# YamaguchiAtsushi/pointcloud_processor

Measured on AMD Instinct MI355X. Metric: ray-hit tests/sec + candidate poses/sec (whole node), 1M-pt terrain, higher is better.
Workload: dtype f64 march / f32 point test; 1 GPU; C2: 1M-pt L-shape excavation terrain, 1024x256 ray fan, 256 candidate poses per GPU; terrain_points=1001740, poses_total=256, num_candidates_lattice=348, parallelism=pose-shard x1

## Files before the change

### include/pcp_abi.h

```cpp
#ifndef PCP_ABI_H
#define PCP_ABI_H

#include <stddef.h>
#include <stdint.h>

#ifdef __cplusplus
extern "C" {
#endif

#define PCP_ABI_VERSION 2

enum pcp_status {
    PCP_OK = 0,
    PCP_E_INVALID = -1,
    PCP_E_HIP = -2,
    PCP_E_CAPACITY = -3,
    PCP_E_STATE = -4,
    PCP_E_NOMEM = -5
};

typedef struct pcp_ctx pcp_ctx;

typedef struct pcp_cloud_view {
    const void *data;
// ... 295 lines not shown
int pcp_step_table(double end, double *steps, uint64_t cap, uint64_t *n);

int pcp_debug_exclusive_scan(pcp_ctx *ctx, const uint32_t *in, uint64_t n, uint32_t *out);

typedef struct pcp_fine_geo {
    int32_t built;
    int32_t tile;
    int32_t skip;
    int32_t packed;
    int32_t nx, ny, nz;
    int32_t F, reach, fnx, fny, rz, tsteps;
    uint64_t n_points, n_records, n_entries;
    uint64_t start_off;
    uint64_t frec_bytes, wpts_bytes, pts_bytes;
    double ox, oy, oz, c, inv_c, r_q;
    double cf, inv_cf, R2;
    double zq;
    double clear_zt0, clear_c;
} pcp_fine_geo;
int pcp_debug_fine_copy(pcp_ctx *ctx, pcp_fine_geo *geo, void *frec, uint64_t frec_cap,
                        void *wpts, uint64_t wpts_cap, void *pts, uint64_t pts_cap);

typedef struct pcp_fine_pivot_geo {
    int32_t built;
    int32_t enabled;
    int32_t fnx, fny;
    int32_t tx, ty;
    uint64_t n_slots;
    uint64_t bytes;
    double ox, oy, cf;
} pcp_fine_pivot_geo;
int pcp_debug_fine_pivot(pcp_ctx *ctx, pcp_fine_pivot_geo *geo, void *piv, uint64_t piv_cap);

typedef struct pcp_index_info {
    uint64_t n_points;
    double cell;
    int32_t nx, ny, nz;
    int32_t fine_pivot;
    double bmin[3], bmax[3];
    int32_t scan_layout;
    int32_t fine_tile;
} pcp_index_info;
int pcp_terrain_info(pcp_ctx *ctx, pcp_index_info *info);

#ifdef __cplusplus
}
#endif
#endif
```

### pointcloud_processor_amd/_abi.py

```python
from __future__ import annotations

import ctypes as C
import os
from pathlib import Path

import numpy as np

_HERE = Path(__file__).resolve().parent
LIB_PATH = _HERE / "_lib" / "libpcp.so"

PCP_OK = 0
PCP_E_INVALID = -1
PCP_E_HIP = -2
PCP_E_CAPACITY = -3
PCP_E_STATE = -4
PCP_E_NOMEM = -5

MAX_STEPS = 4096

PCP_MEM_DEVICE_IN = 1
PCP_MEM_DEVICE_OUT = 2

F_RANGE_Z, F_FOV_Z, F_VIS_Z, F_RANGE_M, F_FOV_M, F_VIS_M = 1, 2, 4, 8, 16, 32

# ... 163 lines not shown
    ("pcp_raycast_fan_stamps", C.c_int, [_P, _P, C.c_uint64, C.POINTER(FanParams), _P]),
    ("pcp_raycast_fan_burst", C.c_int, [_P, _P, C.c_uint64, C.POINTER(FanParams), C.c_int,
                                        C.POINTER(C.c_double)]),
    ("pcp_raycast_fan_keys", C.c_int, [_P, _P, C.c_uint64, C.POINTER(FanParams), C.c_uint64,
                                       C.c_uint64, _P, _P, _P]),
    ("pcp_comm_unique_id", C.c_int, [_P]),
    ("pcp_comm_init_rank", C.c_int, [_P, C.c_int, _P, C.c_int]),
    ("pcp_comm_info", C.c_int, [_P, C.POINTER(C.c_int), C.POINTER(C.c_int)]),
    ("pcp_get_runtime_info", C.c_int, [C.POINTER(RuntimeInfo)]),
    ("pcp_raycast_fan_allreduce", C.c_int, [_P, _P, C.c_uint64, C.POINTER(FanParams), C.c_uint64,
                                            C.c_uint64, _P, _P, C.POINTER(C.c_int64),
                                            C.POINTER(C.c_double)]),
    ("pcp_score_poses_allreduce", C.c_int, [_P, _P, C.c_uint64, _P, C.POINTER(VlParams),
                                            C.c_uint64, C.c_uint64, _P, _P, _P,
                                            C.POINTER(VlReport), C.POINTER(C.c_double)]),
    ("pcp_score_poses_stats", C.c_int, [_P, _P, C.c_uint64, _P, C.POINTER(VlParams), _P]),
    ("pcp_score_matrix", C.c_int, [_P, _P, C.c_uint64, _P, C.POINTER(VlParams), _P, _P]),
    ("pcp_place_sensors", C.c_int, [_P, _P, C.c_uint64, _P, C.POINTER(VlParams),
                                    C.POINTER(PlaceParams), _P, _P, _P, _P, _P, _P, _P, _P, _P]),
    ("pcp_place_pair", C.c_int, [_P, _P, C.c_uint64, _P, C.POINTER(VlParams),
                                 C.POINTER(PairParams), _P, _P, _P, _P, _P, _P, _P, _P, _P, _P,
                                 _P, _P, _P]),
    ("pcp_place_pair_burst", C.c_int, [_P, _P, C.c_uint64, _P, C.POINTER(VlParams),
                                       C.POINTER(PairParams), C.c_int, C.POINTER(C.c_double)]),
    ("pcp_simulate_scan", C.c_int, [_P, _P, C.c_uint64, C.POINTER(FanParams), _P, C.c_uint64,
                                    C.POINTER(C.c_uint64), _P, _P, _P, _P, _P, C.c_uint64,
                                    C.POINTER(C.c_uint64), _P, C.POINTER(C.c_uint64)]),
    ("pcp_simulate_scan_burst", C.c_int, [_P, _P, C.c_uint64, C.POINTER(FanParams), C.c_int,
                                          _P]),
    ("pcp_debug_exclusive_scan", C.c_int, [_P, _P, C.c_uint64, _P]),
    ("pcp_debug_fine_copy", C.c_int, [_P, C.POINTER(FineGeo), _P, C.c_uint64, _P, C.c_uint64, _P,
                                      C.c_uint64]),
    ("pcp_debug_fine_pivot", C.c_int, [_P, C.POINTER(FinePivotGeo), _P, C.c_uint64]),
    ("pcp_score_poses_burst", C.c_int, [_P, _P, C.c_uint64, _P, C.POINTER(VlParams), C.c_int,
                                        C.POINTER(C.c_double)]),
    ("pcp_stream_create", C.c_int, [_P, C.POINTER(_P)]),
    ("pcp_stream_destroy", C.c_int, [_P, _P]),
    ("pcp_step_table", C.c_int, [C.c_double, _P, C.c_uint64, C.POINTER(C.c_uint64)]),
    ("pcp_terrain_info", C.c_int, [_P, C.POINTER(IndexInfo)]),
    ("pcp_multi_create", C.c_int, [C.c_int, _P, C.POINTER(_P)]),
    ("pcp_multi_destroy", None, [_P]),
    ("pcp_multi_last_error", C.c_char_p, [_P]),
    ("pcp_multi_info", C.c_int, [_P, C.POINTER(C.c_int), C.POINTER(C.c_int)]),
    ("pcp_multi_ctx", _P, [_P, C.c_int]),
    ("pcp_multi_set_terrain", C.c_int, [_P, C.POINTER(CloudView)]),
    ("pcp_multi_set_aux_cloud", C.c_int, [_P, C.POINTER(CloudView)]),
    ("pcp_multi_set_cells", C.c_int, [_P, _P, _P, C.c_uint64]),
    ("pcp_multi_raycast_fan", C.c_int, [_P, _P, C.c_uint64, C.POINTER(FanParams), _P, _P,
                                        C.POINTER(C.c_int64)]),
    ("pcp_multi_score_poses", C.c_int, [_P, _P, C.c_uint64, _P, C.POINTER(VlParams), _P, _P,
                                        _P, C.POINTER(VlReport)]),
]
ABI_SYMBOLS = [s[0] for s in _SIGS]

_lib = None


def load_library(path: str | os.PathLike | None = None) -> C.CDLL:
    global _lib
    if _lib is not None and path is None:
        return _lib
    p = Path(path) if path else Path(os.environ.get("PCP_LIB", LIB_PATH))
    if not p.exists():
        raise OSError(f"libpcp.so not found at {p}: run __graft_entry__.build() "
                      f"(make -C pointcloud_processor_amd/csrc)")
    lib = C.CDLL(str(p), mode=C.RTLD_GLOBAL)
# ... 562 lines not shown
    def debug_exclusive_scan(self, a: np.ndarray) -> np.ndarray:
        a = np.ascontiguousarray(a, np.uint32)
        out = np.zeros(a.size + 1, np.uint32)
        self._check(self.lib.pcp_debug_exclusive_scan(self.h, _ptr(a), a.size, _ptr(out)),
                    "pcp_debug_exclusive_scan")
        return out

    def debug_fine_copy(self):
        geo = FineGeo()
        self._check(self.lib.pcp_debug_fine_copy(self.h, C.byref(geo), None, 0, None, 0, None, 0),
                    "pcp_debug_fine_copy")
        d = {k: getattr(geo, k) for k, _ in geo._fields_}
        if not geo.built:
            return d, None, None, None
        frec = np.zeros(geo.frec_bytes, np.uint8)
        wpts = np.zeros(geo.wpts_bytes, np.uint8)
        pts = np.zeros((geo.n_points, 4), np.float32)
        self._check(self.lib.pcp_debug_fine_copy(self.h, C.byref(geo), _ptr(frec), frec.nbytes,
                                                 _ptr(wpts), wpts.nbytes, _ptr(pts), pts.nbytes),
                    "pcp_debug_fine_copy")
        return d, frec, wpts, pts

    def debug_fine_pivot(self):
        geo = FinePivotGeo()
        self._check(self.lib.pcp_debug_fine_pivot(self.h, C.byref(geo), None, 0),
                    "pcp_debug_fine_pivot")
        d = {k: getattr(geo, k) for k, _ in geo._fields_}
        if not geo.built:
            return d, None
        piv = np.zeros((geo.n_slots, 3), np.float32)
        self._check(self.lib.pcp_debug_fine_pivot(self.h, C.byref(geo), _ptr(piv), piv.nbytes),
                    "pcp_debug_fine_pivot")
        return d, piv

    def score_matrix(self, poses5, zx120_pose5, params: VlParams):
        poses = np.ascontiguousarray(poses5, np.float64).reshape(-1, 5)
        zx = np.ascontiguousarray(zx120_pose5, np.float64)
        C_ = self.cells_count()
        P = poses.shape[0]
        sm = np.zeros((max(P, 1), max(C_, 1)), np.float64)
        sz = np.zeros(max(C_, 1), np.float64)
        self._check(self.lib.pcp_score_matrix(self.h, _ptr(poses), P, _ptr(zx), C.byref(params),
                                              _ptr(sm), _ptr(sz)), "pcp_score_matrix")
        return sm[:P, :C_].copy(), sz[:C_].copy()

    def place_sensors(self, poses5, zx120_pose5, params: VlParams, k_max: int,
                      min_separation: float = 0.0, want_round_totals: bool = False,
                      want_cells: bool = False, reserved: int = 0) -> dict:
        poses = np.ascontiguousarray(poses5, np.float64).reshape(-1, 5)
        zx = np.ascontiguousarray(zx120_pose5, np.float64)
        P = poses.shape[0]
        pp = PlaceParams(int(k_max), int(reserved), float(min_separation))
        kk = max(min(int(k_max), PLACE_MAX), 1)
        sel = np.full(kk, -1, np.int64)
        tot = np.zeros(kk, np.float64)
        cov = np.zeros(kk, np.int32)
        rt = np.zeros((kk, max(P, 1)), np.float64) if want_round_totals else None
        C_ = self.cells_count() if want_cells else 0
        cs = np.zeros(max(C_, 1), np.float64) if want_cells else None
        co = np.zeros(max(C_, 1), np.int32) if want_cells else None
        zt, zc, ns = C.c_double(), C.c_int32(), C.c_int32()
        self._check(self.lib.pcp_place_sensors(self.h, _ptr(poses) if P else None, P, _ptr(zx),
                                               C.byref(params), C.byref(pp), _ptr(sel), _ptr(tot),
                                               _ptr(cov), _ptr(rt), _ptr(cs), _ptr(co),
                                               C.byref(zt), C.byref(zc), C.byref(ns)),
                    "pcp_place_sensors")
# ... 310 lines not shown
```

### pointcloud_processor_amd/_stamps.py

```python
from __future__ import annotations

import hashlib
import os
from pathlib import Path

ROOT = Path(__file__).resolve().parents[1]
CSRC = ROOT / "pointcloud_processor_amd" / "csrc"
_COMMON = ["pcp_internal.hpp", "Makefile", "../../include/pcp_abi.h"]
WORKLOAD_SOURCES = {
    "fan": ["pcp_vlidar.hip", "pcp_fine.hip", "pcp_index.hip", "pcp_stencil.hpp",
            "pcp_grid.hpp", "pcp_fan_clear.hpp", "pcp_fan_clip.hpp", "pcp_fan_pivot.hpp"] + _COMMON,
    "filter": ["pcp_filter.hip", "pcp_rigid.hpp"] + _COMMON,
    "cells": ["pcp_vlidar.hip", "pcp_fine.hip", "pcp_index.hip", "pcp_stencil.hpp",
              "pcp_grid.hpp", "pcp_fan_clear.hpp", "pcp_fan_clip.hpp", "pcp_fan_pivot.hpp"] + _COMMON,
}


def workload_stamp(key: str) -> str:
    h = hashlib.sha256(os.environ.get("EXTRA", "").encode())
    for name in WORKLOAD_SOURCES[key]:
        f = (CSRC / name).resolve()
        h.update(name.encode())
        h.update(f.read_bytes())
    return h.hexdigest()[:16]
```

### pointcloud_processor_amd/csrc/pcp_context.hip

```cpp
#include <cmath>
#include <cstdio>
#include <dlfcn.h>
#include <execinfo.h>
#include <cstdarg>
#include <cstdlib>
#include <cstring>
#include <new>

#include "pcp_fan_clip.hpp"
#include "pcp_internal.hpp"

namespace pcp {

int set_err(pcp_ctx *ctx, int code, const char *fmt, ...) {
    if (ctx) {
        char buf[512];
        va_list ap;
        va_start(ap, fmt);
        vsnprintf(buf, sizeof(buf), fmt, ap);
        va_end(ap);
        ctx->err = buf;
    }
    return code;
}
// ... 564 lines not shown
int pcp_alloc_stats(uint64_t *device_reallocs, uint64_t *pinned_reallocs, uint64_t *bytes) {
    if (device_reallocs) *device_reallocs = alloc_count(0);
    if (pinned_reallocs) *pinned_reallocs = alloc_count(1);
    if (bytes) *bytes = alloc_count(2);
    return PCP_OK;
}

int pcp_device_count(int *n) {
    if (!n) return PCP_E_INVALID;
    int c = 0;
    if (hipGetDeviceCount(&c) != hipSuccess) c = 0;
    *n = c;
    return PCP_OK;
}

int pcp_create(int device, pcp_ctx **out) {
    if (!out) return PCP_E_INVALID;
    *out = nullptr;
    int c = 0;
    if (hipGetDeviceCount(&c) != hipSuccess || c <= 0) return PCP_E_HIP;
    if (device < 0 || device >= c) return PCP_E_INVALID;
    if (hipSetDevice(device) != hipSuccess) return PCP_E_HIP;
    pcp_ctx *ctx = new (std::nothrow) pcp_ctx();
    if (!ctx) return PCP_E_NOMEM;
    ctx->device = device;
    if (const char *fb = std::getenv("PCP_FAN_BATCH")) ctx->fan_batch = std::atoi(fb);
    if (const char *fw = std::getenv("PCP_FAN_NPW")) {
        const int v = std::atoi(fw);
        ctx->fan_npw = (v == 2 || v == 4 || v == 8 || v == 16 || v == 32) ? v : 1;
    }
    if (const char *fc = std::getenv("PCP_FAN_CULL")) ctx->fan_cull = std::atoi(fc) != 0;
    if (const char *cl = std::getenv("PCP_FAN_CLEAR")) ctx->terrain.fan_clear = std::atoi(cl) != 0;
    if (const char *pv = std::getenv("PCP_FAN_PIVOT")) ctx->terrain.fan_pivot = std::atoi(pv) != 0;
    if (const char *cp = std::getenv("PCP_FAN_CLIP"))
        ctx->terrain.fan_clip_e = std::atoi(cp) != 0 ? pcp::kClipSlack : pcp::kClipSlackWhole;
    if (const char *fo = std::getenv("PCP_FAN_ORDER")) ctx->fan_horizon_first = std::atoi(fo) != 0;
    if (const char *ho = std::getenv("PCP_FAN_HOST_OUT")) ctx->fan_host_out = std::atoi(ho) != 0;
    if (const char *ne = std::getenv("PCP_NORMALS_EXACT")) ctx->normals_exact = std::atoi(ne) != 0;
    if (const char *sw = std::getenv("PCP_SCORE_WIDE")) ctx->score_wide = std::atoi(sw) != 0;
    if (const char *wr = std::getenv("PCP_SCORE_WIDE_RAYS")) ctx->score_wide_rays = std::atoll(wr);
    if (const char *wg = std::getenv("PCP_SCORE_WIDE_G")) {
        char *end = nullptr;
        const long v = std::strtol(wg, &end, 10);
        if (end == wg || *end != '\0' || !(v == 2 || v == 4 || v == 8 || v == 16)) {
            std::fprintf(stderr, "libpcp: pcp_create: PCP_SCORE_WIDE_G=\"%s\" is not one of 2, 4, 8, 16\n",
                         wg);
            delete ctx;
            return PCP_E_INVALID;
        }
        ctx->score_wide_g = (int)v;
    }
    if (const char *co = std::getenv("PCP_CELLS_ORDER_FREE")) ctx->cells_all_ordered = std::atoi(co) == 0;
    if (const char *nbk = std::getenv("PCP_NB_BLOCKS")) ctx->nb_blocks = std::atoi(nbk);
    if (const char *sp = std::getenv("PCP_SCAN_ONEPASS")) ctx->scan_onepass = std::atoi(sp) != 0;
    if (const char *ip = std::getenv("PCP_INDEX_PAIR")) ctx->index_pair = std::atoi(ip) != 0;
    if (const char *as = std::getenv("PCP_AREA_STREAM")) ctx->area_side = std::atoi(as) != 0;
    if (const char *ns = std::getenv("PCP_NB_SMALL")) ctx->nb_small = std::atoi(ns) != 0;
    if (const char *rp = std::getenv("PCP_NB_REGION_PCT"))
        ctx->nb_region_pct = std::min(100, std::max(1, std::atoi(rp)));
    if (const char *gw = std::getenv("PCP_NB_GUESS_WORDS"))
        ctx->nb_guess_max = std::max<uint64_t>(1, std::strtoull(gw, nullptr, 10));
    if (const char *ct = std::getenv("PCP_COPY_THREADS")) ctx->copy_threads = std::atoi(ct);
    if (const char *fo = std::getenv("PCP_FM_HOST_OUT")) ctx->fm_host_out = std::atoi(fo) != 0;
    if (const char *ff = std::getenv("PCP_FM_FAST")) {
        const int v = std::atoi(ff);
        ctx->fm_fast = (v == 0 || v == 1) ? v : 2;
// ... 214 lines not shown
```

### pointcloud_processor_amd/csrc/pcp_fine.hip

```cpp
#pragma clang fp contract(off)

#include <cfloat>
#include <cmath>

#include <rocprim/device/device_radix_sort.hpp>

#include "pcp_fan_clear.hpp"
#include "pcp_fan_pivot.hpp"
#include "pcp_grid.hpp"
#include "pcp_internal.hpp"

namespace pcp {

namespace {

constexpr int kThreads = 256;

struct FineGeo {
    double ox, oy;
    double cf, inv_cf;
    double R2;
    int32_t fnx, fny;
    int32_t reach;
};

__device__ __forceinline__ bool in_window(const FineGeo &f, double px, double py, int wx, int wy) {
    const double x0 = f.ox + (double)wx * f.cf, y0 = f.oy + (double)wy * f.cf;
    const double dx = fmax(fmax(x0 - px, px - (x0 + f.cf)), 0.0);
    const double dy = fmax(fmax(y0 - py, py - (y0 + f.cf)), 0.0);
    return dx * dx + dy * dy <= f.R2;
}

__device__ __forceinline__ void fine_cell(const FineGeo &f, float x, float y, int &cx, int &cy) {
    cx = min(max((int)floor(((double)x - f.ox) * f.inv_cf), 0), f.fnx - 1);
    cy = min(max((int)floor(((double)y - f.oy) * f.inv_cf), 0), f.fny - 1);
}

__global__ void __launch_bounds__(kThreads)
k_zkeys(const float4 *__restrict__ pts, uint32_t n, unsigned long long *__restrict__ key,
// ... 165 lines not shown
    const uint32_t w = blockIdx.x * kThreads + threadIdx.x;
    if (w >= nw) return;
    const int x = (int)(w % (uint32_t)fnx), y = (int)(w / (uint32_t)fnx);
    uint32_t top = rz;
    for (int d = 0; d <= kClearMax && top > 0u; ++d) {
        const int ya = y - d, yb = y + d;
        const uint32_t la = ya >= 0 ? lev[(size_t)ya * fnx + x] : 0xFFFFFFFFu;
        const uint32_t lb = yb < fny ? lev[(size_t)yb * fnx + x] : 0xFFFFFFFFu;
        const uint32_t m = min(la, lb);
        for (uint32_t iz = m; iz < top; ++iz) h[(size_t)iz * nw + w] = (uint16_t)d;
        top = min(top, m);
    }
    for (uint32_t iz = 0; iz < top; ++iz) h[(size_t)iz * nw + w] = (uint16_t)(kClearMax + 1);
}

__global__ void __launch_bounds__(kThreads)
k_clear_code(const uint16_t *__restrict__ h, int fnx, int fny, uint32_t nw, uint32_t tx,
             size_t plane, uint16_t *__restrict__ fband) {
    const uint32_t w = blockIdx.x * kThreads + threadIdx.x, iz = blockIdx.y;
    if (w >= nw) return;
    const uint32_t wx = w % (uint32_t)fnx, wy = w / (uint32_t)fnx;
    if (fan_clear_border(wx, wy, iz, (uint32_t)fnx, (uint32_t)fny, gridDim.y)) return;
    const size_t r = (size_t)iz * plane + (((size_t)((wy >> 3) * tx + (wx >> 3)) << 6) |
                                           ((wy & 7u) << 3) | (wx & 7u));
    if (fband[r] != 0x00FFu) return;
    const uint16_t *row = h + (size_t)iz * nw + (size_t)wy * fnx;
    int D = (int)row[wx];
    for (int d = 1; d < D; ++d) {
        const int xa = (int)wx - d, xb = (int)wx + d;
        if (xa >= 0) D = min(D, max((int)row[xa], d));
        if (xb < fnx) D = min(D, max((int)row[xb], d));
    }
    fband[r] = (uint16_t)(0x00FFu | (fan_clear_code((uint32_t)D) << 8));
}

__global__ void __launch_bounds__(kThreads)
k_pivot(const float4 *__restrict__ wpts, const uint32_t *__restrict__ cstart, FineGeo f,
        uint32_t tx, uint32_t nslot, float *__restrict__ piv) {
    const uint32_t t = blockIdx.x * kThreads + threadIdx.x;
    if (t >= nslot) return;
    const uint32_t tile = t >> 6, sub = t & 63u;
    const uint32_t wx = (tile % tx) * 8u + (sub & 7u), wy = (tile / tx) * 8u + (sub >> 3);
    float3 best = make_float3(__int_as_float(0x7FC00000), __int_as_float(0x7FC00000), -INFINITY);
    if (wx < (uint32_t)f.fnx && wy < (uint32_t)f.fny) {
        const uint32_t w = wx + (uint32_t)f.fnx * wy;
        const uint32_t s = cstart[w] + w, e = cstart[w + 1] + w;
        PivotKey kb{};
        for (uint32_t j = s; j < e; ++j) {
            const float4 p = wpts[j];
            const PivotKey k{pivot_d2(f.ox, f.oy, f.cf, wx, wy, p.x, p.y), p.z,
                             __float_as_uint(p.w)};
            if (j == s || pivot_better(k, kb)) {
                kb = k;
                best = make_float3(p.x, p.y, p.z);
            }
        }
    }
    float *o = piv + 3 * (size_t)t;
    o[0] = best.x;
    o[1] = best.y;
    o[2] = best.z;
}

__global__ void __launch_bounds__(kThreads)
k_pack3(const float4 *__restrict__ src, uint32_t n, float *__restrict__ dst) {
    const uint32_t i = blockIdx.x * kThreads + threadIdx.x;
// ... 138 lines not shown
    hipLaunchKernelGGL(k_frec, dim3((unsigned)((nthr + kThreads - 1) / kThreads)), dim3(kThreads), 0,
                       st, went, (const uint32_t *)cstart, m, g.c, (uint32_t)fnx,
                       (uint32_t)fny, (uint32_t)rz, tsteps, tile, skip2 ? 1 : 0,
                       g.frec.as<uint2>(),
                       g.frec.as<uint16_t>(),
                       reinterpret_cast<uint32_t *>(g.frec.as<char>() + band_bytes));
    PCP_CHECK_LAUNCH(ctx);
    if (pivots) {
        hipLaunchKernelGGL(k_pivot, dim3((unsigned)((plan.npiv + kThreads - 1) / kThreads)),
                           dim3(kThreads), 0, st, (const float4 *)went, (const uint32_t *)cstart,
                           f, pivot_tiles((uint32_t)fnx), (uint32_t)plan.npiv,
                           g.fpiv.as<float>());
        PCP_CHECK_LAUNCH(ctx);
    }
    if (tile == 2) {
        const size_t lev_bytes = ((size_t)nw * 4 + 255) & ~(size_t)255;
        PCP_HIP(ctx, ctx->scratch[5].ensure(lev_bytes + (size_t)nw * rz * 2 + 64));
        uint32_t *lev = ctx->scratch[5].as<uint32_t>();
        uint16_t *hcol = reinterpret_cast<uint16_t *>(ctx->scratch[5].as<char>() + lev_bytes);
        const ClearGeo cg = plan.cg;
        PCP_HIP(ctx, hipMemsetAsync(lev, 0xFF, (size_t)nw * 4, st));
        hipLaunchKernelGGL(k_clear_level, dim3(gridn), dim3(kThreads), 0, st, pts, n, f, cg,
                           (int)rz, lev);
        PCP_CHECK_LAUNCH(ctx);
        const dim3 cgrid((unsigned)((nw + kThreads - 1) / kThreads), (unsigned)rz);
        hipLaunchKernelGGL(k_clear_col, dim3(cgrid.x), dim3(kThreads), 0, st,
                           (const uint32_t *)lev, (int)fnx, (int)fny, (uint32_t)nw, (uint32_t)rz,
                           hcol);
        PCP_CHECK_LAUNCH(ctx);
        hipLaunchKernelGGL(k_clear_code, cgrid, dim3(kThreads), 0, st, (const uint16_t *)hcol,
                           (int)fnx, (int)fny, (uint32_t)nw, (uint32_t)((fnx + 7) / 8), (size_t)(nrec / rz),
                           g.frec.as<uint16_t>());
        PCP_CHECK_LAUNCH(ctx);
    }
    if (pack) {
        hipLaunchKernelGGL(k_pack3, dim3((unsigned)((nent + kThreads - 1) / kThreads)),
                           dim3(kThreads), 0, st, (const float4 *)went, (uint32_t)nent,
                           g.wpts.as<float>());
        PCP_CHECK_LAUNCH(ctx);
    }
    g.wpack = pack ? 1 : 0;
    g.frx = (uint32_t)fnx;
    g.fry = (uint32_t)fny;
    g.frz = (uint32_t)rz;
    g.ffine = (float)F;
    g.ftile = tile;
    g.fskip = skip2 ? 2 : 1;
    g.fstart_off = tile == 2 ? band_bytes : 0;
    g.fnent = nent;
    g.fpiv_ok = pivots;
    g.fine_ok = true;
    return PCP_OK;
}

}

extern "C" int pcp_debug_fine_copy(pcp_ctx *ctx, pcp_fine_geo *geo, void *frec,
                                   uint64_t frec_cap, void *wpts, uint64_t wpts_cap, void *pts,
                                   uint64_t pts_cap) {
    using namespace pcp;
    if (!ctx || !geo) return PCP_E_INVALID;
    const GridIndex &g = ctx->terrain;
    *geo = pcp_fine_geo{};
    if (!g.present || !g.fine_ok) return PCP_OK;
    const FinePlan p = fine_plan(g, (int)g.ffine, g.ftile);
    geo->built = 1;
// ... 37 lines not shown
    if (frec) PCP_HIP(ctx, hipMemcpy(frec, g.frec.p, geo->frec_bytes, hipMemcpyDeviceToHost));
    if (wpts) PCP_HIP(ctx, hipMemcpy(wpts, g.wpts.p, geo->wpts_bytes, hipMemcpyDeviceToHost));
    if (pts) PCP_HIP(ctx, hipMemcpy(pts, g.pts.p, geo->pts_bytes, hipMemcpyDeviceToHost));
    return PCP_OK;
}

extern "C" int pcp_debug_fine_pivot(pcp_ctx *ctx, pcp_fine_pivot_geo *geo, void *piv,
                                    uint64_t piv_cap) {
    using namespace pcp;
    if (!ctx || !geo) return PCP_E_INVALID;
    const GridIndex &g = ctx->terrain;
    *geo = pcp_fine_pivot_geo{};
    if (!g.present || !g.fine_ok || !g.fpiv_ok) return PCP_OK;
    const FinePlan p = fine_plan(g, (int)g.ffine, g.ftile);
    geo->built = 1;
    geo->enabled = g.fan_pivot ? 1 : 0;
    geo->fnx = p.f.fnx;
    geo->fny = p.f.fny;
    geo->tx = (int32_t)pivot_tiles((uint32_t)p.fnx);
    geo->ty = (int32_t)pivot_tiles((uint32_t)p.fny);
    geo->n_slots = p.npiv;
    geo->bytes = p.npiv * kPivotBytes;
    geo->ox = p.f.ox;
    geo->oy = p.f.oy;
    geo->cf = p.f.cf;
    if (!piv) return PCP_OK;
    if (piv_cap < geo->bytes)
        return set_err(ctx, PCP_E_CAPACITY, "pcp_debug_fine_pivot: the buffer is too small");
    PCP_HIP(ctx, hipSetDevice(ctx->device));
    PCP_HIP(ctx, hipStreamSynchronize(ctx->stream));
    PCP_HIP(ctx, hipMemcpy(piv, g.fpiv.p, geo->bytes, hipMemcpyDeviceToHost));
    return PCP_OK;
}
```

### pointcloud_processor_amd/csrc/pcp_index.hip

```cpp
#include <cfloat>
#include <cmath>
#include <cstring>

#include "pcp_internal.hpp"
#include "pcp_grid.hpp"

namespace pcp {

constexpr uint64_t kMaxCells = 1ull << 25;
constexpr int kThreads = 256;

GridView GridIndex::view() const {
    GridView v{};
    v.pts = pts.as<const float4>();
    v.start = start.as<const uint32_t>();
    v.occ2 = occ2_ok ? occ2.as<const uint32_t>() : nullptr;
    v.c = c;
    v.inv_c = c > 0 ? 1.0 / c : 0.0;
    v.ox = bmin[0] - c;
    v.oy = bmin[1] - c;
    v.oz = bmin[2] - c;
    const double rm = r_q + kQueryMargin;
    double amax = 0.0;
    for (int a = 0; a < 3; ++a) amax = fmax(amax, fmax(fabs(bmin[a]), fabs(bmax[a])));
// ... 2 lines not shown
    v.lo_y = v.oy + rm;
    v.lo_z = v.oz + rm;
    v.nx = nx;
    v.ny = ny;
    v.nz = nz;
    v.n_pts = (uint32_t)n_pts;
    v.bx0 = bmin[0] - rb;
    v.bx1 = bmax[0] + rb;
    v.by0 = bmin[1] - rb;
    v.by1 = bmax[1] + rb;
    v.bz0 = bmin[2] - rb;
    v.bz1 = bmax[2] + rb;
    v.flo_x = (float)v.lo_x;
    v.flo_y = (float)v.lo_y;
    v.flo_z = (float)v.lo_z;
    v.finv_c = (float)v.inv_c;
    v.fnx1 = (float)(nx - 1);
    v.fny1 = (float)(ny - 1);
    v.fnz1 = (float)(nz - 1);
    const double bb[6] = {v.bx0, v.bx1, v.by0, v.by1, v.bz0, v.bz1};
    for (int a = 0; a < 6; ++a) v.fb[a] = (float)bb[a];
    v.occz = occz_ok ? occz.as<const uint16_t>() : nullptr;
    v.bstart = blk_ok ? bstart.as<const uint32_t>() : nullptr;
    v.bpts = blk_ok ? bpts.as<const float4>() : nullptr;
    v.fzoff = (float)(rm * v.inv_c);
    v.fzt = (float)((r_q + 2e-3) * v.inv_c);
    v.frec = fine_ok ? frec.as<const uint2>() : nullptr;
    v.wpts = fine_ok ? wpts.as<const float4>() : nullptr;
    v.frx = fine_ok ? frx : 0u;
    v.fry = fine_ok ? fry : 0u;
    v.frz = fine_ok ? frz : 0u;
    v.ffine = fine_ok ? ffine : 0.0f;
    v.ftile = fine_ok ? ftile : 0;
    v.fband = (fine_ok && ftile == 2) ? frec.as<const uint16_t>() : nullptr;
    v.fzc = (float)c;
    v.wpack = fine_ok ? wpack : 0;
    v.fzo = (float)v.oz;
    v.fstart = (fine_ok && ftile == 2)
                   ? reinterpret_cast<const uint32_t *>(frec.as<const char>() + fstart_off)
                   : nullptr;
    v.fus_off = (float)(rm * v.inv_c / (double)kZq);
    v.fskip = fine_ok ? fskip : 1;
    v.fclear = (fine_ok && ftile == 2 && fan_clear) ? 1 : 0;
    v.fclr_cf = fine_ok ? (float)(c / (double)ffine) : 0.0f;
    v.fclr_rb = std::nextafter((float)rb, INFINITY);
    const bool piv = fine_ok && ftile == 2 && fpiv_ok;
    v.fpiv = (piv && fan_pivot) ? fpiv.as<const float>() : nullptr;
    v.fptx = piv ? (frx + 7u) >> 3 : 0u;
    v.fpty = piv ? (fry + 7u) >> 3 : 0u;
    v.fclip_e = fan_clip_e;
    return v;
}

float exit_dist(float r2) {
    float d = std::sqrt(r2);
    while (d * d < r2) d = std::nextafter(d, INFINITY);
    for (float p = std::nextafter(d, 0.0f); p * p >= r2; p = std::nextafter(d, 0.0f)) d = p;
    return d;
}

__device__ __forceinline__ float ld_f32(const unsigned char *base, uint32_t off) {
    return *reinterpret_cast<const float *>(base + off);
}

__global__ void __launch_bounds__(kThreads)
k_extract(const unsigned char *__restrict__ raw, uint64_t n, uint32_t step, uint32_t ox,
          uint32_t oy, uint32_t oz, float4 *__restrict__ xyz, float *__restrict__ part,
// ... 510 lines not shown
    PCP_HIP(ctx, ctx->scratch[4].ensure(scan_tmp_bytes(ncm) + (ncm + 1) * sizeof(uint32_t)));
    if (int rc = exclusive_scan_u32_pair(ctx, cnt_a, ga.start.as<uint32_t>(), nca, cnt_a, cnt_b,
                                         gb.start.as<uint32_t>(), ncb, cnt_b, ctx->scratch[4].p,
                                         true))
        return rc;
    ctx->cell_cnt_dirty = ctx->cell_cnt2_dirty = false;
    PCP_HIP(ctx, ga.pts.ensure((size_t)nfin * sizeof(float4)));
    PCP_HIP(ctx, gb.pts.ensure((size_t)nfin * sizeof(float4)));
    hipLaunchKernelGGL(k_cell_place2, dim3(gridn), dim3(kThreads), 0, st,
                       ctx->scratch[0].as<const float4>(), n, (const uint2 *)cr_a,
                       ga.start.as<const uint32_t>(), ga.pts.as<float4>(), (const uint2 *)cr_b,
                       gb.start.as<const uint32_t>(), gb.pts.as<float4>());
    PCP_CHECK_LAUNCH(ctx);
    ga.present = gb.present = true;
    *paired = true;
    return PCP_OK;
}

int build_index(pcp_ctx *ctx, GridIndex &g, const pcp_cloud_view &v, double r_q, bool zsort,
                bool occ, const unsigned char **raw_io, unsigned char *raw_copy) {
    const uint64_t n = v.n;
    hipStream_t st = ctx->stream;
    if (n >= (1ull << 28))
        return set_err(ctx, PCP_E_INVALID, "index cloud of %llu points exceeds 2^28",
                       (unsigned long long)n);
    ProfScope prof(ctx, PCP_K_INDEX_BUILD);
    g.present = false;
    g.occz_ok = false;
    g.occ2_ok = false;
    g.blk_ok = false;
    g.blk_fail = false;
    g.fine_ok = false;
    g.fpiv_ok = false;
    g.fine_fail = false;
    const uint64_t raw_bytes = n * (uint64_t)v.point_step;
    const unsigned char *raw = raw_io ? *raw_io : nullptr;
    bool pinned = false;
    if (!raw && n && ctx->zc_in && raw_bytes <= kPinDirectMax) {
        const HostPiece pc{0, v.data, raw_bytes};
        const void *dv = nullptr;
        if (int rc0 = pin_stage(ctx, &pc, 1, raw_bytes, &dv)) return rc0;
        raw = static_cast<const unsigned char *>(dv);
        pinned = true;
    }
    if (!raw) {
        PCP_HIP(ctx, ctx->stage.ensure(raw_bytes));
        if (int rc0 = upload_async(ctx, ctx->stage.p, v.data, raw_bytes, st)) return rc0;
        raw = ctx->stage.as<unsigned char>();
    }
    const bool host_bb = n <= kHostBboxMax;
    const bool fuse_copy = raw_copy && host_bb && n && (v.point_step & 15u) == 0 &&
                           v.point_step <= 64 &&
                           ((reinterpret_cast<uintptr_t>(raw) | reinterpret_cast<uintptr_t>(raw_copy)) & 15u) == 0;
    if (raw_copy && n && !fuse_copy) {
        if (int rc0 = copy_pinned_async(ctx, raw_copy, raw, raw_bytes, st)) return rc0;
        raw = raw_copy;
    }
    if (raw_io) *raw_io = raw_copy && n ? raw_copy : raw;
    auto release_raw = [&]() {
        if (pinned && !raw_io) pin_release(ctx, st);
    };
    const int nb = (int)std::min<uint64_t>((n + kThreads - 1) / kThreads, 1024);
    PCP_HIP(ctx, ctx->scratch[0].ensure(n * sizeof(float4)));
    PCP_HIP(ctx, ctx->scratch[1].ensure((size_t)nb * 6 * sizeof(float) + 64 + nb * 4));
    PCP_HIP(ctx, ctx->stats_d.ensure(64));
    float *part = ctx->scratch[1].as<float>();
// ... 225 lines not shown
```

### pointcloud_processor_amd/csrc/pcp_internal.hpp

```cpp
#pragma once

#include <hip/hip_runtime.h>

#include <algorithm>
#include <atomic>
#include <cstdint>
#include <cstdio>
#include <string>
#include <vector>

#include "pcp_abi.h"
#include "pcp_fan_pick.hpp"

namespace pcp {
struct CopyPool;

constexpr double kPi = 3.14159265358979323846;
constexpr double kMinDistance = 0.5;
constexpr double kRayStep = 0.3;
constexpr double kVisRadius = 0.08;
constexpr double kRayRadius = kVisRadius * 0.7;
constexpr double kRelaxedRadius = kVisRadius * 3.0;
constexpr double kMinElevation = -85.0 * kPi / 180.0;
constexpr double kMaxElevation = 85.0 * kPi / 180.0;
// ... 65 lines not shown
    double bx0, bx1, by0, by1, bz0, bz1;
    float flo_x, flo_y, flo_z, finv_c;
    float fnx1, fny1, fnz1;
    float fb[6];
    const uint16_t *occz;
    float fzoff, fzt;
    const uint32_t *bstart;
    const float4 *bpts;
    const uint2 *frec;
    const float4 *wpts;
    uint32_t frx, fry, frz;
    float fus_off, ffine;
    int32_t ftile;
    const uint16_t *fband;
    const uint32_t *fstart;
    int32_t fskip;
    float fzc, fzo;
    int32_t wpack;
    int32_t fclear;
    float fclr_cf, fclr_rb;
    const float *fpiv;
    uint32_t fptx, fpty;
    float fclip_e;
};
constexpr float kZq = 2.0f / 250.0f;

struct GridIndex {
    bool present = false;
    uint64_t n_pts = 0;
    double r_q = 0.0;
    double c = 0.0;
    int32_t nx = 0, ny = 0, nz = 0;
    double bmin[3] = {0, 0, 0}, bmax[3] = {0, 0, 0};
    DevBuf pts, start, occ2, occz, bstart, bpts, frec, wpts, fpiv;
    bool occz_ok = false;
    bool blk_ok = false;
    bool blk_fail = false;
    bool fine_ok = false;
    bool fine_fail = false;
    uint32_t frx = 0, fry = 0, frz = 0;
    int32_t wpack = 0;
    float ffine = 0.0f;
    int32_t ftile = 0;
    int32_t fskip = 1;
    bool fan_clear = true;
    bool fpiv_ok = false;
    bool fan_pivot = true;
    float fan_clip_e = 1.0f / 64.0f;
    size_t fstart_off = 0;
    uint64_t fnent = 0;
    bool occ2_ok = false;
    GridView view() const;
    void release() {
        pts.release();
        start.release();
        occ2.release();
        occz.release();
        bstart.release();
        bpts.release();
        frec.release();
        wpts.release();
        fpiv.release();
        fpiv_ok = false;
        occz_ok = false;
        blk_ok = false;
        blk_fail = false;
        fine_ok = false;
        fine_fail = false;
        occ2_ok = false;
        present = false;
        n_pts = 0;
    }
};

struct ProfSlot {
    double total_ms = 0.0;
    uint64_t launches = 0;
};

struct CloudBufs {
    DevBuf xyz, idx, keys[2], sparse, sparse_idx, hist, out;
    DevBuf skeys;
    void release() {
        skeys.release();
        xyz.release();
        idx.release();
        for (int q = 0; q < 2; ++q) keys[q].release();
        sparse.release();
        sparse_idx.release();
        hist.release();
        out.release();
    }
};

struct PendingEvent {
    int kid;
// ... 289 lines not shown
```

Before: 7180 billion ray-hit tests/s.

## Build per-column tight z-band table so fan rays skip empty z slices

Adds a build-time kernel that, for each fine column and z layer, computes the actual z extent that points can reach within the query radius. It stores the narrowed band in a second buffer, which the ray-march view uses in place of the coarse band when enabled (on by default). Tighter bands should let the ray test skip more z sub-steps per cell. The cost is extra index-build work and memory, and the result is only correct if the band margin (rho + mu) is conservative enough.

```diff
diff --git a/include/pcp_abi.h b/include/pcp_abi.h
--- a/include/pcp_abi.h
+++ b/include/pcp_abi.h
@@ -351,6 +351,9 @@
 } pcp_fine_pivot_geo;
 int pcp_debug_fine_pivot(pcp_ctx *ctx, pcp_fine_pivot_geo *geo, void *piv, uint64_t piv_cap);
 
+int pcp_debug_fine_band(pcp_ctx *ctx, uint64_t *bytes, int32_t *enabled, void *band,
+                        uint64_t band_cap);
+
 typedef struct pcp_index_info {
     uint64_t n_points;
     double cell;
diff --git a/pointcloud_processor_amd/_abi.py b/pointcloud_processor_amd/_abi.py
--- a/pointcloud_processor_amd/_abi.py
+++ b/pointcloud_processor_amd/_abi.py
@@ -219,6 +219,8 @@
     ("pcp_debug_fine_copy", C.c_int, [_P, C.POINTER(FineGeo), _P, C.c_uint64, _P, C.c_uint64, _P,
                                       C.c_uint64]),
     ("pcp_debug_fine_pivot", C.c_int, [_P, C.POINTER(FinePivotGeo), _P, C.c_uint64]),
+    ("pcp_debug_fine_band", C.c_int, [_P, C.POINTER(C.c_uint64), C.POINTER(C.c_int32), _P,
+                                      C.c_uint64]),
     ("pcp_score_poses_burst", C.c_int, [_P, _P, C.c_uint64, _P, C.POINTER(VlParams), C.c_int,
                                         C.POINTER(C.c_double)]),
     ("pcp_stream_create", C.c_int, [_P, C.POINTER(_P)]),
@@ -847,6 +849,17 @@
         self._check(self.lib.pcp_debug_fine_pivot(self.h, C.byref(geo), _ptr(piv), piv.nbytes),
                     "pcp_debug_fine_pivot")
         return d, piv
+
+    def debug_fine_band(self):
+        nbytes, enabled = C.c_uint64(), C.c_int32()
+        self._check(self.lib.pcp_debug_fine_band(self.h, C.byref(nbytes), C.byref(enabled), None, 0),
+                    "pcp_debug_fine_band")
+        if not nbytes.value:
+            return int(enabled.value), None
+        band = np.zeros(nbytes.value // 2, np.uint16)
+        self._check(self.lib.pcp_debug_fine_band(self.h, C.byref(nbytes), C.byref(enabled),
+                                                 _ptr(band), band.nbytes), "pcp_debug_fine_band")
+        return int(enabled.value), band
 
     def score_matrix(self, poses5, zx120_pose5, params: VlParams):
         poses = np.ascontiguousarray(poses5, np.float64).reshape(-1, 5)
diff --git a/pointcloud_processor_amd/_stamps.py b/pointcloud_processor_amd/_stamps.py
--- a/pointcloud_processor_amd/_stamps.py
+++ b/pointcloud_processor_amd/_stamps.py
@@ -9,10 +9,12 @@
 _COMMON = ["pcp_internal.hpp", "Makefile", "../../include/pcp_abi.h"]
 WORKLOAD_SOURCES = {
     "fan": ["pcp_vlidar.hip", "pcp_fine.hip", "pcp_index.hip", "pcp_stencil.hpp",
-            "pcp_grid.hpp", "pcp_fan_clear.hpp", "pcp_fan_clip.hpp", "pcp_fan_pivot.hpp"] + _COMMON,
+            "pcp_grid.hpp", "pcp_fan_band.hpp", "pcp_fan_clear.hpp", "pcp_fan_clip.hpp",
+            "pcp_fan_pivot.hpp"] + _COMMON,
     "filter": ["pcp_filter.hip", "pcp_rigid.hpp"] + _COMMON,
     "cells": ["pcp_vlidar.hip", "pcp_fine.hip", "pcp_index.hip", "pcp_stencil.hpp",
-              "pcp_grid.hpp", "pcp_fan_clear.hpp", "pcp_fan_clip.hpp", "pcp_fan_pivot.hpp"] + _COMMON,
+              "pcp_grid.hpp", "pcp_fan_band.hpp", "pcp_fan_clear.hpp", "pcp_fan_clip.hpp",
+              "pcp_fan_pivot.hpp"] + _COMMON,
 }
 
 
diff --git a/pointcloud_processor_amd/csrc/pcp_context.hip b/pointcloud_processor_amd/csrc/pcp_context.hip
--- a/pointcloud_processor_amd/csrc/pcp_context.hip
+++ b/pointcloud_processor_amd/csrc/pcp_context.hip
@@ -620,6 +620,7 @@
     if (const char *fc = std::getenv("PCP_FAN_CULL")) ctx->fan_cull = std::atoi(fc) != 0;
     if (const char *cl = std::getenv("PCP_FAN_CLEAR")) ctx->terrain.fan_clear = std::atoi(cl) != 0;
     if (const char *pv = std::getenv("PCP_FAN_PIVOT")) ctx->terrain.fan_pivot = std::atoi(pv) != 0;
+    if (const char *bd = std::getenv("PCP_FAN_BAND")) ctx->terrain.fan_band = std::atoi(bd) != 0;
     if (const char *cp = std::getenv("PCP_FAN_CLIP"))
         ctx->terrain.fan_clip_e = std::atoi(cp) != 0 ? pcp::kClipSlack : pcp::kClipSlackWhole;
     if (const char *fo = std::getenv("PCP_FAN_ORDER")) ctx->fan_horizon_first = std::atoi(fo) != 0;
diff --git a/pointcloud_processor_amd/csrc/pcp_fan_band.hpp b/pointcloud_processor_amd/csrc/pcp_fan_band.hpp
--- /dev/null
+++ b/pointcloud_processor_amd/csrc/pcp_fan_band.hpp
@@ -0,0 +1,50 @@
+#pragma once
+
+#include <cmath>
+#include <cstdint>
+
+#if defined(__HIPCC__)
+#define PCP_BAND_HD __host__ __device__ inline
+#else
+#define PCP_BAND_HD inline
+#endif
+
+namespace pcp {
+
+constexpr double kBandMu = 2e-3;
+
+struct BandAcc {
+    double top, bottom;
+    bool any;
+};
+
+PCP_BAND_HD BandAcc fan_band_begin() { return BandAcc{-INFINITY, INFINITY, false}; }
+
+PCP_BAND_HD double fan_band_dist(double ox, double oy, double cf, int wx, int wy, double px,
+                                 double py) {
+    const double x0 = ox + (double)wx * cf, y0 = oy + (double)wy * cf;
+    const double dx = fmax(fmax(x0 - px, px - (x0 + cf)), 0.0);
+    const double dy = fmax(fmax(y0 - py, py - (y0 + cf)), 0.0);
+    return sqrt(dx * dx + dy * dy);
+}
+
+PCP_BAND_HD void fan_band_add(BandAcc &a, double z, double d, double m, double rho) {
+    const double g = fmax(d - m, 0.0);
+    if (!(g < rho)) return;
+    const double reach = sqrt(rho * rho - g * g);
+    a.top = fmax(a.top, z + reach);
+    a.bottom = fmin(a.bottom, z - reach);
+    a.any = true;
+}
+
+PCP_BAND_HD uint32_t fan_band_word(const BandAcc &a, double zb, double step, uint32_t spec) {
+    if (!a.any) return 254u;
+    const double h = ceil((a.top - zb) / step) + 1.0;
+    const double l = floor((a.bottom - zb) / step) - 1.0;
+    const uint32_t hi = h >= 255.0 ? 255u : (uint32_t)fmax(h, 1.0);
+    const uint32_t lo = l <= 0.0 ? 0u : (uint32_t)fmin(l, 254.0);
+    const uint32_t slo = spec & 255u, shi = (spec >> 8) & 255u;
+    return (lo > slo ? lo : slo) | ((hi < shi ? hi : shi) << 8);
+}
+
+}
diff --git a/pointcloud_processor_amd/csrc/pcp_fine.hip b/pointcloud_processor_amd/csrc/pcp_fine.hip
--- a/pointcloud_processor_amd/csrc/pcp_fine.hip
+++ b/pointcloud_processor_amd/csrc/pcp_fine.hip
@@ -5,6 +5,7 @@
 
 #include <rocprim/device/device_radix_sort.hpp>
 
+#include "pcp_fan_band.hpp"
 #include "pcp_fan_clear.hpp"
 #include "pcp_fan_pivot.hpp"
 #include "pcp_grid.hpp"
@@ -236,6 +237,45 @@
         if (xb < fnx) D = min(D, max((int)row[xb], d));
     }
     fband[r] = (uint16_t)(0x00FFu | (fan_clear_code((uint32_t)D) << 8));
+}
+
+__global__ void __launch_bounds__(kThreads)
+k_band_tight(const float4 *__restrict__ wpts, const uint32_t *__restrict__ cstart, CellMap m,
+             FineGeo f, double c, double qm, double rho, uint32_t rz, uint32_t tx, size_t plane,
+             const uint16_t *__restrict__ fband, uint16_t *__restrict__ twin) {
+    const uint32_t nw = (uint32_t)f.fnx * (uint32_t)f.fny, w = blockIdx.x * kThreads + threadIdx.x;
+    if (w >= nw) return;
+    const uint32_t wx = w % (uint32_t)f.fnx, wy = w / (uint32_t)f.fnx;
+    const size_t base = ((size_t)((wy >> 3) * tx + (wx >> 3)) << 6) | ((wy & 7u) << 3) | (wx & 7u);
+    const uint32_t s = cstart[w] + w, e = cstart[w + 1] + w;
+    uint32_t jt = s, jb = s;
+    int ct = s < e ? cell_z(m, wpts[s].z) : -1, cb = ct;
+    const double step = (double)kZq * c;
+    for (int iz = (int)rz - 1; iz >= 0; --iz) {
+        while (jt < e && ct > iz + 1) {
+            ++jt;
+            ct = jt < e ? cell_z(m, wpts[jt].z) : -1;
+        }
+        if (jb < jt) {
+            jb = jt;
+            cb = ct;
+        }
+        while (jb < e && cb >= iz) {
+            ++jb;
+            cb = jb < e ? cell_z(m, wpts[jb].z) : -1;
+        }
+        const size_t r = (size_t)iz * plane + base;
+        const uint32_t spec = fband[r];
+        if (jb == jt || (spec & 255u) == 255u) continue;
+        BandAcc a = fan_band_begin();
+        for (uint32_t j = jt; j < jb; ++j) {
+            const float4 p = wpts[j];
+            fan_band_add(a, (double)p.z,
+                         fan_band_dist(f.ox, f.oy, f.cf, (int)wx, (int)wy, (double)p.x, (double)p.y),
+                         qm, rho);
+        }
+        twin[r] = (uint16_t)fan_band_word(a, m.oz + (double)iz * c, step, spec);
+    }
 }
 
 __global__ void __launch_bounds__(kThreads)
@@ -440,6 +480,21 @@
                            (int)fnx, (int)fny, (uint32_t)nw, (uint32_t)((fnx + 7) / 8), (size_t)(nrec / rz),
                            g.frec.as<uint16_t>());
         PCP_CHECK_LAUNCH(ctx);
+        g.fband_ok = false;
+        if (g.fband2.ensure(band_bytes) == hipSuccess) {
+            PCP_HIP(ctx, hipMemcpyAsync(g.fband2.p, g.frec.p, band_bytes, hipMemcpyDeviceToDevice,
+                                        st));
+            hipLaunchKernelGGL(k_band_tight, dim3(cgrid.x), dim3(kThreads), 0, st,
+                               (const float4 *)went, (const uint32_t *)cstart, m, f, g.c,
+                               kQueryMargin, g.r_q + kBandMu, (uint32_t)rz,
+                               (uint32_t)((fnx + 7) / 8), (size_t)(nrec / rz),
+                               g.frec.as<const uint16_t>(), g.fband2.as<uint16_t>());
+            PCP_CHECK_LAUNCH(ctx);
+            g.fband_ok = true;
+        } else {
+            (void)hipGetLastError();
+            g.fband2.release();
+        }
     }
     if (pack) {
         hipLaunchKernelGGL(k_pack3, dim3((unsigned)((nent + kThreads - 1) / kThreads)),
@@ -543,3 +598,22 @@
     PCP_HIP(ctx, hipMemcpy(piv, g.fpiv.p, geo->bytes, hipMemcpyDeviceToHost));
     return PCP_OK;
 }
+
+extern "C" int pcp_debug_fine_band(pcp_ctx *ctx, uint64_t *bytes, int32_t *enabled, void *band,
+                                   uint64_t band_cap) {
+    using namespace pcp;
+    if (!ctx || !bytes) return PCP_E_INVALID;
+    const GridIndex &g = ctx->terrain;
+    *bytes = 0;
+    if (enabled) *enabled = g.fan_band ? 1 : 0;
+    if (!g.present || !g.fine_ok || !g.fband_ok) return PCP_OK;
+    const FinePlan p = fine_plan(g, (int)g.ffine, g.ftile);
+    *bytes = (uint64_t)p.nrec * 2;
+    if (!band) return PCP_OK;
+    if (band_cap < *bytes)
+        return set_err(ctx, PCP_E_CAPACITY, "pcp_debug_fine_band: the buffer is too small");
+    PCP_HIP(ctx, hipSetDevice(ctx->device));
+    PCP_HIP(ctx, hipStreamSynchronize(ctx->stream));
+    PCP_HIP(ctx, hipMemcpy(band, g.fband2.p, *bytes, hipMemcpyDeviceToHost));
+    return PCP_OK;
+}
diff --git a/pointcloud_processor_amd/csrc/pcp_index.hip b/pointcloud_processor_amd/csrc/pcp_index.hip
--- a/pointcloud_processor_amd/csrc/pcp_index.hip
+++ b/pointcloud_processor_amd/csrc/pcp_index.hip
@@ -58,7 +58,9 @@
     v.frz = fine_ok ? frz : 0u;
     v.ffine = fine_ok ? ffine : 0.0f;
     v.ftile = fine_ok ? ftile : 0;
-    v.fband = (fine_ok && ftile == 2) ? frec.as<const uint16_t>() : nullptr;
+    v.fband = !(fine_ok && ftile == 2) ? nullptr
+              : (fband_ok && fan_band)   ? fband2.as<const uint16_t>()
+                                         : frec.as<const uint16_t>();
     v.fzc = (float)c;
     v.wpack = fine_ok ? wpack : 0;
     v.fzo = (float)v.oz;
@@ -635,6 +637,7 @@
     g.blk_fail = false;
     g.fine_ok = false;
     g.fpiv_ok = false;
+    g.fband_ok = false;
     g.fine_fail = false;
     const uint64_t raw_bytes = n * (uint64_t)v.point_step;
     const unsigned char *raw = raw_io ? *raw_io : nullptr;
diff --git a/pointcloud_processor_amd/csrc/pcp_internal.hpp b/pointcloud_processor_amd/csrc/pcp_internal.hpp
--- a/pointcloud_processor_amd/csrc/pcp_internal.hpp
+++ b/pointcloud_processor_amd/csrc/pcp_internal.hpp
@@ -121,7 +121,7 @@
     double c = 0.0;
     int32_t nx = 0, ny = 0, nz = 0;
     double bmin[3] = {0, 0, 0}, bmax[3] = {0, 0, 0};
-    DevBuf pts, start, occ2, occz, bstart, bpts, frec, wpts, fpiv;
+    DevBuf pts, start, occ2, occz, bstart, bpts, frec, wpts, fpiv, fband2;
     bool occz_ok = false;
     bool blk_ok = false;
     bool blk_fail = false;
@@ -135,6 +135,8 @@
     bool fan_clear = true;
     bool fpiv_ok = false;
     bool fan_pivot = true;
+    bool fband_ok = false;
+    bool fan_band = true;
     float fan_clip_e = 1.0f / 64.0f;
     size_t fstart_off = 0;
     uint64_t fnent = 0;
@@ -150,7 +152,9 @@
         frec.release();
         wpts.release();
         fpiv.release();
+        fband2.release();
         fpiv_ok = false;
+        fband_ok = false;
         occz_ok = false;
         blk_ok = false;
         blk_fail = false;
```

Measured after the change: 7466 billion ray-hit tests/s (median of 6 runs). +4.0%, better.
